# c-f-h/pyiga

Measured on AMD Instinct MI355X. Metric: assembled elements/sec (3D p=4, 128^3 spans) + HBM-roofline %; 1/2/4/8 GPU, higher is better.
Workload: dtype f64

## Files before the change

include/igx.h:

```cpp
#ifndef IGX_H
#define IGX_H

#include <stddef.h>
#include <stdint.h>

#ifdef __cplusplus
extern "C" {
#endif

#define IGX_VERSION 101
#define IGX_MAX_DIM 3
#define IGX_MAX_DEGREE 15
#define IGX_MAX_SF_DEGREE 7

typedef struct igx_ctx igx_ctx;
typedef struct igx_patch igx_patch;
typedef struct igx_multipatch igx_multipatch;

enum { IGX_MASS = 0, IGX_STIFFNESS = 1,
       IGX_CONVDIFF = 2,
       IGX_FORM = 3 };
enum { IGX_GEO_BSPLINE = 0, IGX_GEO_NURBS = 1, IGX_GEO_JACOBIAN = 2 };
enum { IGX_ALGO_AUTO = 0,
       IGX_ALGO_ENTRYWISE = 1,
// ... 21 lines not shown
    const double *gauss_w;

    int32_t row0_lo, row0_hi;

    int32_t box_lo[IGX_MAX_DIM], box_hi[IGX_MAX_DIM];
} igx_patch_desc;

typedef struct {
    int32_t dim, nqp;
    int32_t ndofs[IGX_MAX_DIM], nspans[IGX_MAX_DIM], ngauss[IGX_MAX_DIM];
    int64_t nrows_total;
    int64_t row_lo, row_hi;
    int64_t nnz;
    int64_t nnz_offset;
    int64_t nelem_owned;
    int32_t sumfact_ok;
    int32_t reserved;
} igx_patch_info;

typedef struct {
    float total_ms;
    float fields_ms, stage0_ms, stage1_ms, final_ms, entry_ms;
    int32_t algo_used;
    int32_t n_launches;
} igx_timing;

#define IGX_PATH_GEOA    1
#define IGX_PATH_FUSED   2
#define IGX_PATH_MIRROR  4
#define IGX_PATH_SINGLE  8
#define IGX_PATH_BOTH   32
#define IGX_PATH_BF3    64
#define IGX_PATH_TWIN  128
#define IGX_PATH_KRON   16

int         igx_version(void);
const char *igx_last_error(void);

igx_ctx *igx_create(int device_id);
void     igx_destroy(igx_ctx *ctx);
int      igx_sync(igx_ctx *ctx);
void    *igx_stream(igx_ctx *ctx);

int igx_active_deriv(igx_ctx *ctx, const double *kv, int kv_len, int p,
                     const double *u, size_t nu, int numderiv, double *out);
int igx_find_spans(igx_ctx *ctx, const double *kv, int kv_len, int p,
                   const double *u, size_t nu, int64_t *spans);

int igx_grid_jacobian(igx_ctx *ctx, const igx_patch_desc *desc, int ncomp,
                      const double *const grid[IGX_MAX_DIM], const int32_t ngrid[IGX_MAX_DIM],
                      double *jac_out, double *eval_out);

igx_patch *igx_patch_create(igx_ctx *ctx, const igx_patch_desc *desc);
void       igx_patch_destroy(igx_patch *patch);
int        igx_patch_get_info(const igx_patch *patch, igx_patch_info *info);

int igx_patch_set_coeff(igx_patch *patch, const double *coeff);
int igx_patch_set_coeff_affine(igx_patch *patch, const double c[4]);

int igx_patch_set_coeff_expr(igx_patch *patch, const char *expr, int *cache_hit);

int igx_patch_eval_expr_d(igx_patch *patch, const char *expr, int parametric, double *d_out, int *cache_hit);

int igx_rtc_compile(const char *expr, const char *arch, char *path_out, int path_len, int *cache_hit);

int igx_patch_set_form(igx_patch *patch, const double *const coef[16]);
// ... 397 lines not shown
```

pyiga_amd/assemblers.py:

```python
import os
import ctypes as C
import weakref

import numpy as np
import scipy.sparse

from . import _lib
from . import bspline
from .quadrature import make_tensor_quadrature
from . import geometry

_ENTRY_TRAMPOLINES = []


def _is_spline_geo(geo):
    return hasattr(geo, 'kvs') and hasattr(geo, 'coeffs') and hasattr(geo, 'sdim')


def _is_nurbs(geo):
    from .geometry import NurbsFunc
    return isinstance(geo, NurbsFunc) or type(geo).__name__ == 'NurbsFunc'


class DevicePatch:
# ... 211 lines not shown
            _lib.check(lib.igx_patch_add_face(self.handle, int(axis), int(side), face.handle), 'igx_patch_add_face')
        else:
            vals = _lib.f64(face).ravel()
            _lib.check(lib.igx_patch_add_face_host(self.handle, int(axis), int(side), _lib.dptr(vals), C.c_int64(vals.size)),
                       'igx_patch_add_face_host')

    def assemble_kron(self, kind, patch2, m0, k0=None, to_host=True):
        out = np.empty(self.nnz) if to_host else None
        m0 = _lib.f64(m0)
        k0 = None if k0 is None else _lib.f64(k0)
        _lib.check(_lib.load().igx_assemble_kron3(self.handle, patch2.handle, _lib.KINDS[kind], _lib.dptr(m0),
                                                  None if k0 is None else _lib.dptr(k0), _lib.dptr(out) if to_host else None),
                   'igx_assemble_kron3')
        return out

    def fast_assemble(self, kind, tol=1e-10, maxiter=100, skipcount=3, tolcount=3, verbose=0, batch=None):
        assert self.row_range == (0, self.shape[0]), 'the low-rank assembler works on whole patches'
        lib = _lib.load()
        if batch is not None:
            _lib.check(lib.igx_patch_set_aca_batch(self.handle, int(batch)), 'igx_patch_set_aca_batch')
        data = np.empty(self.nnz)
        rank, nent, nreq = C.c_int(0), C.c_longlong(0), C.c_longlong(0)
        _lib.check(lib.igx_fast_assemble(self.handle, _lib.KINDS[kind], float(tol), int(maxiter), int(skipcount), int(tolcount),
                                         int(verbose), _lib.dptr(data), C.byref(rank), C.byref(nent)), 'igx_fast_assemble')
        _lib.check(lib.igx_fast_assemble_stats(self.handle, C.byref(nreq), None, None), 'igx_fast_assemble_stats')
        self.aca_stats = {'rank': rank.value, 'entries': nent.value, 'requests': nreq.value, 'nnz': int(self.nnz)}
        indptr, indices = self.pattern()
        return scipy.sparse.csr_matrix((data, indices, indptr), shape=self.shape)

    def last_path(self):
        bits = _lib.load().igx_patch_last_path(self.handle)
        return {name for bit, name in ((1, 'geoA'), (2, 'fused'), (4, 'mirror'), (8, 'single'), (16, 'kron'), (32, 'both'), (64, 'bf3'), (128, 'twin')) if bits & bit}

    def fields_plan(self, kind):
        out = (C.c_int64 * 4)()
        _lib.check(_lib.load().igx_patch_fields_plan(self.handle, _lib.KINDS[kind], out), 'igx_patch_fields_plan')
        return {'lines': bool(out[0]), 'lpb': int(out[1]), 'lds': int(out[2]), 'nc': int(out[3])}

    def single2d_plan(self, kind, whole_patch=False):
        out = (C.c_int64 * 9)()
        _lib.check(_lib.load().igx_patch_single2d_plan(self.handle, _lib.KINDS[kind], 1 if whole_patch else 0, out), 'igx_patch_single2d_plan')
        names = ('supported', 'wanted', 'R0', 'R1', 'NG0', 'WIN', 'NCOL', 'lds', 'blocks')
        d = {n: int(v) for n, v in zip(names, out)}
        d['supported'], d['wanted'] = bool(d['supported']), bool(d['wanted'])
        return d

    def placement(self):
        n, b, w = C.c_int(0), C.c_float(0), C.c_float(0)
        _lib.check(_lib.load().igx_patch_placement(self.handle, C.byref(n), C.byref(b), C.byref(w)), 'igx_patch_placement')
        return {'tried': n.value, 'best_ms': round(b.value, 4), 'worst_ms': round(w.value, 4)}

    def timing(self):
        t = _lib.Timing()
        _lib.check(_lib.load().igx_last_timing(self.handle, C.byref(t)), 'igx_last_timing')
        return t.as_dict()

    def entries(self, kind, idx):
        idx = np.ascontiguousarray(idx, dtype=np.uintp)
        assert idx.ndim == 2 and idx.shape[1] == 2
        out = np.zeros(idx.shape[0])
        _lib.check(_lib.load().igx_entries(self.handle, _lib.KINDS[kind], idx.ctypes.data_as(C.POINTER(C.c_size_t)),
                                           idx.shape[0], _lib.dptr(out)), 'igx_entries')
        return out

    def fields(self, kind):
        shp = (C.c_int64 * 4)()
# ... 885 lines not shown
```

pyiga_amd/csrc/geoa.hip:

```cpp
#include <cstdlib>
#include <cstdio>
#include <algorithm>
#include "geo_device.h"

namespace igx {

constexpr int GA_MAXS = 8;
#ifndef GA_ONEDIV
#define GA_ONEDIV 1
#endif
#ifndef GA_SPREAD
#define GA_SPREAD 0
#endif
#ifndef GA_READBOTH
#define GA_READBOTH 1
#endif
#ifndef GA_DPP
#define GA_DPP 1
#endif
typedef const double __attribute__((address_space(4))) *cdp;
typedef const int __attribute__((address_space(4))) *cip;

struct GeoAArgs {
    GeoView gv;
    const double *w0, *w1, *w2;
    int nurbs, kind;
    int G1, G2;
    long long NPL, stride;
    const double *tab;
    const int *steps;
    int s_lo, s_hi, q, chunk_len;
    int ntiles;
#ifdef IGX_ABLATE
    int dbg;
#endif
    int field[GA_MAXS], type[GA_MAXS];
    double *out[GA_MAXS];
    int xfield[GA_MAXS], xtype[GA_MAXS];
    const double *coeff;
    int g0_lo, coef_affine;
    double cf[4];
    int soff_ok;
    double pc[16];
    const double *pa[16];
    int pmask, amask, fmask;
    int fslot[16];
    int nsrc[GA_MAXS], sfield[GA_MAXS][4], stype[GA_MAXS][4];
    int nslots;
    int nodiag[GA_MAXS];
};
constexpr int GA_NFT = 13;

typedef int int8v __attribute__((ext_vector_type(8)));

#ifdef IGX_ABLATE
#define GA_OFF(bit) (A.dbg & (bit))
#else
#define GA_OFF(bit) false
#endif

#ifdef IGX_GA_STAMP
__device__ unsigned long long g_ga_stamp[2048 * 8 * 6];
#define GA_T(i) do { const unsigned long long n_ = __builtin_amdgcn_s_memtime(); st_[i] += n_ - st_t; st_t = n_; } while (0)
#else
#define GA_T(i)
#endif

template <int M>
__device__ __forceinline__ void fmac_rowbc(double &acc, const double pv, const double bv)
{
    asm("v_fmac_f64_dpp %0, %1, %2 row_newbcast:%3 row_mask:0xf bank_mask:0xf" : "+v"(acc) : "v"(pv), "v"(bv), "n"(M));
}
template <int P, int A_ = 0, int B_ = 0>
__device__ __forceinline__ void sweep_lower_rowbc(double (&acc)[P][P], const double (&pv)[(P * (P + 1) / 2 + 15) / 16], const double bv)
{
    if constexpr (A_ < P) {
        constexpr int m = A_ * (A_ + 1) / 2 + B_;
        fmac_rowbc<(m & 15)>(acc[A_][B_], pv[m >> 4], bv);
        if constexpr (B_ < A_) sweep_lower_rowbc<P, A_, B_ + 1>(acc, pv, bv);
        else sweep_lower_rowbc<P, A_ + 1, 0>(acc, pv, bv);
    }
}

template <int P, int M = 0>
__device__ __forceinline__ void sweep_full_rowbc(double (&acc)[P][P], const double (&pv)[(P * P + 15) / 16], const double bv)
{
    if constexpr (M < P * P) {
        fmac_rowbc<(M & 15)>(acc[M / P][M % P], pv[M >> 4], bv);
        sweep_full_rowbc<P, M + 1>(acc, pv, bv);
    }
}

constexpr int GA_REC = 42;
constexpr int GA_ROWS = 16;

__global__ void k_geoa_table(const double *V0s, int P, const double *V0g, const int *fa0g, int P0G, const double *w0, int q,
                             const int *step_ptr, const int *steps, int G0, double *tab, const int *rows, int nonsym)
{
    const int g = blockIdx.x * blockDim.x + threadIdx.x;
    if (g >= G0) return;
    double *r = tab + (size_t)g * GA_REC;
    for (int k = 0; k < GA_REC; ++k) r[k] = 0.0;
    for (int a = 0; a < P; ++a) { r[a] = V0s[((size_t)g * P + a) * 2]; r[6 + a] = V0s[((size_t)g * P + a) * 2 + 1]; }
    for (int e = 0; e < 2 * P0G; ++e) r[12 + e] = V0g[(size_t)g * P0G * 2 + e];
    r[18] = w0[g];
    r[19] = (double)fa0g[g];
    int *ri = (int *)(r + 20);
    const int s = g / q;
    if (g - s * q == q - 1) {
        const int st0 = step_ptr[s], st1 = step_ptr[s + 1];
        ri[0] = st1 - st0; ri[1] = st0;
        if (st1 > st0 && !nonsym)
            for (int a = 0; a < P; ++a) ri[2 + a] = steps[(size_t)st0 * 8 + a];
    }
    int *ra = (int *)(r + 24), *rs = (int *)(r + 32), *rb = (int *)(r + 40);
    for (int m = 0; m < GA_ROWS; ++m) { ra[m] = 0; rs[m] = -1; }
    rb[0] = 0; rb[1] = 0;
    if (nonsym) {
        if (g - s * q == q - 1 && step_ptr[s + 1] > step_ptr[s])
            for (int m = 0; m < 16; ++m) ra[m] = steps[(size_t)step_ptr[s] * 16 + m];
    } else if (rows) {
        const int *sr = rows + (size_t)s * (2 * GA_ROWS + 2);
        for (int m = 0; m < GA_ROWS; ++m) ra[m] = sr[m];
        if (g - s * q == q - 1) {
            for (int m = 0; m < GA_ROWS; ++m) rs[m] = sr[GA_ROWS + m];
            rb[0] = sr[2 * GA_ROWS];
        }
    }
}

struct K1Store {
    __amdgpu_buffer_rsrc_t rs;
    int voff, ok;
    int voffd, nodiag;
    __device__ __forceinline__ K1Store(double *base, const long long pt, const int tile, const int soff_ok, const int nodiag_ = 0)
    {
        const long long t0 = (long long)tile * 64;
        rs = __builtin_amdgcn_make_buffer_rsrc((void *)(base + t0), (short)0, 0x7ffffff0, 0x00020000);
        voff = (int)(pt - t0) * 8;
        nodiag = nodiag_;
        voffd = nodiag_ ? 0x7ffffff8 : voff;
#ifdef GA_K1_FLAT
        ok = 0;
#else
        ok = soff_ok;
#endif
    }
    __device__ __forceinline__ void store(double *out, const int slot, const long long stride, const double x) const
    {
        if (ok) {
            typedef int i2s __attribute__((ext_vector_type(2)));
            i2s v; v.x = __double2loint(x); v.y = __double2hiint(x);
            __builtin_amdgcn_raw_buffer_store_b64(v, rs, voff, (int)((unsigned)slot * (unsigned)(stride * 8)), 0);
        } else out[(long long)slot * stride] = x;
    }
    __device__ __forceinline__ void store_diag(double *out, const int slot, const long long stride, const double x) const
    {
        if (ok) {
            typedef int i2s __attribute__((ext_vector_type(2)));
            i2s v; v.x = __double2loint(x); v.y = __double2hiint(x);
            __builtin_amdgcn_raw_buffer_store_b64(v, rs, voffd, (int)((unsigned)slot * (unsigned)(stride * 8)), 0);
        } else if (!nodiag) out[(long long)slot * stride] = x;
// ... 769 lines not shown
            __syncthreads();
        }
        return;
    }
    if constexpr (DPS) {
        const bool live = w < A.nslots;
        const int t = A.type[w], fi = A.field[w];
        double *const out = A.out[w] + pt;
        const K1Store k1s(A.out[w], pt, tile, A.soff_ok, D2 ? 0 : A.nodiag[w]);
        double acc[P][P];
#pragma unroll
        for (int a = 0; a < P; ++a)
#pragma unroll
            for (int b = 0; b < P; ++b) acc[a][b] = 0.0;
        auto products = [&](const int rsl, const int bufn) {
            for (int i = tid; i < NS * 64; i += NT) {
                const int jp = i >> 6, ty = (i >> 4) & 3, m = i & 15;
                const int a = m >= 10 ? 4 : m >= 6 ? 3 : m >= 3 ? 2 : m >= 1 ? 1 : 0, b = m - a * (a + 1) / 2;
                const double x = rec[rsl][jp][6 * (ty >> 1) + a] * rec[rsl][jp][6 * (ty & 1) + b];
                prd_[((bufn * NS + jp) * 4 + ty) * 16 + m] = m < NPR ? x : 0.0;
            }
        };
        const double *const pw = &prd_[t * 16 + (lane & 15)];
#ifdef IGX_GA_STAMP
        unsigned long long st_[6] = {0, 0, 0, 0, 0, 0}, st_t = __builtin_amdgcn_s_memtime();
#endif
        stage_load(g_begin); stage_store(0);
        stage_load(g_begin + NS); stage_store(1);
        __syncthreads();
        next_batch(g_begin, 0, 0);
        products(0, 0);
        __syncthreads();
        GA_T(0);
        int it = 0, l = 0, sp = s_begin, rs = 0;
        for (int gb = g_begin; gb < g_end; gb += NS, ++it) {
            const int buf = it & 1;
            const int rn = rs == 2 ? 0 : rs + 1, ra = rn == 2 ? 0 : rn + 1;
            stage_load(gb + 2 * NS);
            double pv[1] = {pw[(buf * NS) * 64]};
            double bv = FLD(buf, 0, fi, lane);
#pragma unroll
            for (int j = 0; j < NS; ++j) {
                if (gb + j >= g_end || !live) break;
                const int jn = j + 1 < NS ? j + 1 : j;
                const double pvn = pw[(buf * NS + jn) * 64], bvn = FLD(buf, jn, fi, lane);
                asm volatile("" ::: "memory");
                if (!GA_OFF(4)) sweep_lower_rowbc<P>(acc, pv, bv);
                else acc[0][0] += pv[0] + bv;
#pragma unroll
                for (int a = 0; a < P; ++a)
#pragma unroll
                    for (int b = 0; b <= a; ++b) asm volatile("" : "+v"(acc[a][b]));
                asm volatile("" ::: "memory");
                pv[0] = pvn; bv = bvn;
                GA_T(1);
                if (++l < q) continue;
                const bool write = sp >= own_lo && !GA_OFF(2);
                const int *fr = (const int *)&rec[rs][j][20];
                const int nst = __builtin_amdgcn_readfirstlane(fr[0]), st0 = __builtin_amdgcn_readfirstlane(fr[1]);
                for (int st = st0; st < st0 + nst; ++st) {
                    int pr[P];
                    if (st == st0) {
#pragma unroll
                        for (int a = 0; a < P; ++a) pr[a] = __builtin_amdgcn_readfirstlane(fr[2 + a]);
                    } else {
                        const int8v rec8 = *(const int8v __attribute__((address_space(4))) *)((cip)A.steps + (size_t)st * 8);
#pragma unroll
                        for (int a = 0; a < P; ++a) pr[a] = rec8[a];
                    }
                    if (pr[0] >= 0 && write) k1s.store_diag(out, pr[0], A.stride, acc[0][0]);
#pragma unroll
                    for (int a = 1; a < P; ++a)
                        if (pr[a] >= 0 && write) k1s.store(out, pr[a], A.stride, acc[a][0]);
#pragma unroll
                    for (int a = 0; a < P - 1; ++a)
#pragma unroll
                        for (int b = 0; b <= a; ++b) acc[a][b] = acc[a + 1][b + 1];
#pragma unroll
                    for (int b = 0; b < P; ++b) acc[P - 1][b] = 0.0;
                }
                l = 0; ++sp;
                GA_T(2);
            }
            GA_T(1);
            next_batch(gb + NS, rn, buf ^ 1);
            products(rn, buf ^ 1);
            GA_T(0);
            stage_store(ra);
            rs = rn;
            __syncthreads();
            GA_T(3);
        }
#ifdef IGX_GA_STAMP
        if (lane == 0 && blockIdx.x < 2048 && blockIdx.y == 0)
            for (int i = 0; i < 4; ++i) g_ga_stamp[(blockIdx.x * 8 + (w & 7)) * 6 + i] = st_[i];
#endif
        return;
    }
    const int t = A.type[w], fi = A.field[w];
    double *const out = A.out[w] + pt;
    const K1Store k1s(A.out[w], pt, tile, A.soff_ok);
    double acc[P][P];
#pragma unroll
    for (int a = 0; a < P; ++a)
#pragma unroll
        for (int b = 0; b < P; ++b) acc[a][b] = 0.0;
#if GA_SPREAD
    double park[P];
    int pslot[P];
    bool have = false;
#pragma unroll
    for (int a = 0; a < P; ++a) { park[a] = 0.0; pslot[a] = -1; }
#endif
    typedef double d2 __attribute__((ext_vector_type(2)));
    const int tu = t & 1, tv = t >> 1;
    auto basis_row = [&](double (&v)[PV], const int buf, const int j, const int d) {
        const d2 *row = (const d2 *)&rec[buf][j][6 * d];
#pragma unroll
        for (int k = 0; k < P / 2; ++k) { const d2 x = row[k]; v[2 * k] = x.x; v[2 * k + 1] = x.y; }
        if (P & 1) v[P - 1] = rec[buf][j][6 * d + P - 1];
    };

#ifdef IGX_GA_STAMP
    unsigned long long st_[6] = {0, 0, 0, 0, 0, 0}, st_t = __builtin_amdgcn_s_memtime();
#endif
// ... 75 lines not shown
                if (nst == 1 && gb + j + 1 < g_end) {
#pragma unroll
                    for (int a = 0; a < P; ++a) { park[a] = acc[a][0]; pslot[a] = write ? pr[a] : -1; }
                    have = true;
                } else
#endif
#pragma unroll
                for (int a = 0; a < P; ++a)
                    if (pr[a] >= 0 && write) k1s.store(out, pr[a], A.stride, acc[a][0]);
#pragma unroll
                for (int a = 0; a < P - 1; ++a)
#pragma unroll
                    for (int b = 0; b <= a; ++b) acc[a][b] = acc[a + 1][b + 1];
#pragma unroll
                for (int b = 0; b < P; ++b) acc[P - 1][b] = 0.0;
            }
            l = 0; ++sp;
            GA_T(2);
        }
        GA_T(1);
        next_batch(gb + NS, rn, buf ^ 1);
        GA_T(0);
        stage_store(ra);
        rs = rn;
        __syncthreads();
        GA_T(3);
    }
#ifdef IGX_GA_STAMP
    if (lane == 0 && blockIdx.x < 2048 && blockIdx.y == 0)
        for (int i = 0; i < 4; ++i) g_ga_stamp[(blockIdx.x * 8 + (w & 7)) * 6 + i] = st_[i];
#endif
}

template <int P, int NS, int P0G>
static int launch_geoA_2d(hipStream_t st, const GeoAArgs &A, int nc, dim3 grid)
{
    if (nc == 3) k_geoA<P, NS, P0G, 3, false, 0, true><<<grid, dim3(geoa_threads(NS, 0)), 0, st>>>(A);
    else k_geoA<P, NS, P0G, 2, false, 0, true><<<grid, dim3(geoa_threads(NS, 0)), 0, st>>>(A);
    IGX_HIP(hipGetLastError());
    return IGX_OK;
}

template <int P, int NS, int P0G, bool MF = false, int FORM = 0>
static int launch_geoA_k(hipStream_t st, const GeoAArgs &A, int nc, dim3 grid)
{
    if (nc == 4) k_geoA<P, NS, P0G, 4, MF, FORM><<<grid, dim3(geoa_threads(NS, FORM)), 0, st>>>(A);
    else k_geoA<P, NS, P0G, 3, MF, FORM><<<grid, dim3(geoa_threads(NS, FORM)), 0, st>>>(A);
    IGX_HIP(hipGetLastError());
#ifdef IGX_GA_STAMP
    {
        static std::vector<unsigned long long> h(2048 * 8 * 6);
        IGX_HIP(hipStreamSynchronize(st));
        IGX_HIP(hipMemcpyFromSymbol(h.data(), HIP_SYMBOL(g_ga_stamp), h.size() * sizeof(unsigned long long)));
        const int nb = std::min<unsigned>(grid.x, 2048);
        for (int w = 0; w < NS; ++w) {
            double t[4] = {0, 0, 0, 0};
            for (int b = 0; b < nb; ++b) for (int i = 0; i < 4; ++i) t[i] += h[(b * 8 + w) * 6 + i];
            fprintf(stderr, "k_geoA stamp: wave %d  geometry %.0f  sweep %.0f  flush %.0f  barrier %.0f  (x100 ns per block)\n", w, t[0] / nb, t[1] / nb, t[2] / nb, t[3] / nb);
        }
    }
#endif
    return IGX_OK;
}

template <int P, int NS>
static int launch_geoA_g(hipStream_t st, const GeoAArgs &A, int nc, int p0g, dim3 grid)
// ... 109 lines not shown
        hipError_t e = hipGetLastError();
        if (e == hipSuccess) e = hipStreamSynchronize(st);
        (void)hipFree(d_rows);
        if (e != hipSuccess) {
            (void)hipFree(tab);
            set_error("per-plane table of the fused geometry + axis-0 sweep: %s", hipGetErrorString(e));
            return IGX_ERR_HIP;
        }
        pt->d_geoa_tab = tab;
        pt->geoa_mf = mf_ok ? 1 : 0;
    }
    GeoAArgs A{};
    const bool d2 = pt->dim == 2;
    A.gv = make_view(pt->dim, pt->gax, pt->d_ctrl, pt->ncomp);
    A.w0 = pd.ax[0].w; A.w1 = pd.ax[1].w; A.w2 = d2 ? nullptr : pd.ax[2].w;
    A.nurbs = pt->geo_kind == IGX_GEO_NURBS; A.kind = kind;
    A.G1 = pd.ax[1].G; A.G2 = d2 ? 1 : pd.ax[2].G;
    A.NPL = (long long)A.G1 * A.G2; A.stride = slice_stride;
    A.soff_ok = (long long)(nonsym ? pt->npairs0n : pt->npairs0) * slice_stride * 8 + 1024 < 0x7ffffff0LL ? 1 : 0;
    A.tab = nonsym ? pt->d_geoa_tabn : pt->d_geoa_tab; A.steps = nonsym ? pt->d_stepsn : pt->stepA_rec;
    A.coeff = pt->d_coeff; A.g0_lo = pd.g0_lo; A.coef_affine = pt->coef_affine;
    for (int k = 0; k < 4; ++k) A.cf[k] = pt->coef_c[k];
    A.s_lo = pt->s0_lo; A.s_hi = pt->s0_hi; A.q = A0.q; A.chunk_len = chunk_len;
#ifdef IGX_ABLATE
    { const char *e = getenv("IGX_GEOA_DBG"); A.dbg = e ? atoi(e) : 0; }
#endif
    for (int x = 0; x < nslots; ++x) {
        A.field[x] = slot_field ? slot_field[x] : 0; A.type[x] = slot_type ? slot_type[x] : 0; A.out[x] = slot_out[x];
        A.xfield[x] = slot_xfield ? slot_xfield[x] : -1; A.xtype[x] = slot_xtype ? slot_xtype[x] : 0;
        A.nodiag[x] = (nodiag_mask >> x) & 1;
    }
    if (nodiag_mask && (nonsym || form || pt->dim != 3 || !geoA_diag_types_commute(pt))) { set_error("internal: diagonal slices skipped on a sweep that does not repeat them"); return IGX_ERR_UNSUPPORTED; }
    A.nslots = nslots;
    for (int x = nslots; x < GA_MAXS; ++x) A.out[x] = A.out[0];
    A.ntiles = (int)((A.NPL + 63) / 64);
    dim3 grid((unsigned)((A.ntiles + 7) / 8 * 8), nchunks);
    const int nc = pt->ncomp, p0g = pt->gax[0].P;
    if (d2) {
#define GEOA_2D(PV) case PV: return nslots == 1 ? (p0g == 2 ? launch_geoA_2d<PV, 1, 2>(st, A, nc, grid) : launch_geoA_2d<PV, 1, 3>(st, A, nc, grid)) \
                                                : (p0g == 2 ? launch_geoA_2d<PV, 4, 2>(st, A, nc, grid) : launch_geoA_2d<PV, 4, 3>(st, A, nc, grid))
        switch (A0.P) { GEOA_2D(2); GEOA_2D(3); GEOA_2D(4); GEOA_2D(5); }
#undef GEOA_2D
        set_error("fused geometry + stage A (2D): unsupported degree %d", A0.p);
        return IGX_ERR_UNSUPPORTED;
    }
    if (form) {
        for (int k = 0; k < 16; ++k) { A.pc[k] = form->pc[k]; A.pa[k] = form->pa[k]; A.fslot[k] = form->fslot[k]; }
        A.pmask = form->pmask; A.nslots = nslots; A.amask = 0; A.fmask = 0;
        for (int k = 0; k < 16; ++k) { if (form->pa[k]) A.amask |= 1 << k; if (form->fslot[k] >= 0) A.fmask |= 1 << k; }
        for (int x = 0; x < GA_MAXS; ++x) {
            A.nsrc[x] = x < nslots ? form->nsrc[x] : 1;
            for (int k = 0; k < 4; ++k) { A.sfield[x][k] = x < nslots ? form->sfield[x][k] : 0; A.stype[x][k] = x < nslots ? form->stype[x][k] : 0; }
            if (x >= nslots) A.out[x] = A.out[0];
        }
#define GEOA_T(PV, FV) case PV: return p0g == 2 ? launch_geoA_k<PV, 8, 2, false, FV>(st, A, nc, grid) : p0g == 3 ? launch_geoA_k<PV, 8, 3, false, FV>(st, A, nc, grid) : IGX_ERR_UNSUPPORTED
        if (form->sym) switch (A0.P) { GEOA_T(3, 3); GEOA_T(4, 3); GEOA_T(5, 3); GEOA_T(6, 3); }
        else switch (A0.P) { GEOA_T(3, 2); GEOA_T(4, 2); GEOA_T(5, 2); GEOA_T(6, 2); }
#undef GEOA_T
        set_error("fused geometry + stage A (general form): unsupported degree %d", A0.p);
        return IGX_ERR_UNSUPPORTED;
    }
    if (nonsym) {
#define GEOA_N(PV) case PV: return p0g == 2 ? launch_geoA_k<PV, 8, 2, false, 1>(st, A, nc, grid) : p0g == 3 ? launch_geoA_k<PV, 8, 3, false, 1>(st, A, nc, grid) : IGX_ERR_UNSUPPORTED
        switch (A0.P) {
            GEOA_N(3); GEOA_N(4); GEOA_N(5); GEOA_N(6);
        }
#undef GEOA_N
        set_error("fused geometry + stage A (non-symmetric): unsupported degree %d", A0.p);
        return IGX_ERR_UNSUPPORTED;
    }
    if (nslots == 8 && pt->geoa_mf && pt->knobs.geoa_mf && (A0.P == 5 || A0.P == 4) && A0.q == A0.P && p0g == 2) {
        if (A0.P == 5) return launch_geoA_k<5, 8, 2, true>(st, A, nc, grid);
        return launch_geoA_k<4, 8, 2, true>(st, A, nc, grid);
    }
#define GEOA_P(PV) case PV: return (nslots == 1 && !(GA_MASS8 && PV <= 5)) ? launch_geoA_g<PV, 1>(st, A, nc, p0g, grid) : launch_geoA_g<PV, 8>(st, A, nc, p0g, grid)
    switch (A0.P) {
        GEOA_P(2); GEOA_P(3); GEOA_P(4); GEOA_P(5); GEOA_P(6);
    }
#undef GEOA_P
    set_error("fused geometry + stage A: unsupported degree %d", A0.p);
    return IGX_ERR_UNSUPPORTED;
}

}
```

pyiga_amd/csrc/igx_api.hip:

```cpp
#include "igx_internal.h"
#include <algorithm>
#include <cmath>
#include <cstdarg>
#include <cstdio>
#include <cstdlib>
#include <cstring>
#include <new>

namespace igx {

static thread_local char g_err[1024] = "";

void set_error(const char *fmt, ...)
{
    va_list ap;
    va_start(ap, fmt);
    vsnprintf(g_err, sizeof(g_err), fmt, ap);
    va_end(ap);
}

static void gauss_legendre(int n, std::vector<double> &x, std::vector<double> &w)
{
    x.assign(n, 0.0);
    w.assign(n, 0.0);
// ... 355 lines not shown
    (void)hipSetDevice(pt->ctx->device);
    (void)hipStreamSynchronize(pt->ctx->stream);
    for (int k = 0; k < 3; ++k) { free_axis(pt->ax[k]); free_geo_axis(pt->gax[k]); }
    (void)hipFree(pt->d_ctrl); (void)hipFree(pt->d_jac); (void)hipFree(pt->d_coeff); (void)hipFree(pt->d_formc); (void)hipFree(pt->d_fields); (void)hipFree(pt->d_data);
    (void)hipFree(pt->ftab_arr);
    (void)hipFree(pt->d_indices); (void)hipFree(pt->d_indptr); (void)hipFree(pt->d_pl0); (void)hipFree(pt->d_rl0_of); (void)hipFree(pt->d_steps); (void)hipFree(pt->d_ldesc);
    (void)hipFree(pt->d_pl0n); (void)hipFree(pt->d_stepsn); (void)hipFree(pt->d_qdesc); (void)hipFree(pt->d_qdescn);
    (void)hipFree(pt->d_K1); (void)hipFree(pt->d_K2);
    (void)hipFree(pt->d_geoa_tab); (void)hipFree(pt->d_geoa_tabn); (void)hipFree(pt->d_zeros); (void)hipFree(pt->d_triv); (void)hipFree(pt->d_tpairs);
    (void)hipFree(pt->d_ws_ij); (void)hipFree(pt->d_ws_out);
    (void)hipFree(pt->d_lv_f); (void)hipFree(pt->d_lv_t1); (void)hipFree(pt->d_lv_t2); (void)hipFree(pt->d_lv_o);
    (void)hipFree(pt->d_sp_ws);
    (void)hipFree(pt->d_q_ws);
    delete pt;
}

igx_patch *igx_patch_create(igx_ctx *ctx, const igx_patch_desc *d)
{
    if (!ctx || !d) { set_error("igx_patch_create: null argument"); return nullptr; }
    const int dim = d->dim;
    if (dim != 2 && dim != 3) { set_error("igx_patch_create: dim must be 2 or 3 (got %d)", dim); return nullptr; }
    if (hipSetDevice(ctx->device) != hipSuccess) { set_error("hipSetDevice failed"); return nullptr; }
    igx_patch *pt = new (std::nothrow) igx_patch();
    if (pt) {
        igx_knobs &k = pt->knobs;
        if (const char *e = getenv("IGX_PATH")) k.path = !strcmp(e, "fused") ? 1 : !strcmp(e, "unfused") ? 2 : !strcmp(e, "single") ? 3 : 0;
        if (const char *e = getenv("IGX_GEOA")) { k.geoa = strcmp(e, "0") != 0; k.geoa_mf = strcmp(e, "mfma") == 0; }
        if (const char *e = getenv("IGX_FINAL")) k.final_sel = !strcmp(e, "q") ? 1 : !strcmp(e, "valu") ? 2 : !strcmp(e, "mfma") ? 3 : 1;
        if (const char *e = getenv("IGX_ENTRIES")) k.entries_thread = !strcmp(e, "thread");
        k.poison = getenv("IGX_DEBUG_POISON") != nullptr;
        if (const char *e = getenv("IGX_BF")) k.bf = atoi(e);
        k.no_twin = getenv("IGX_NO_TWIN") != nullptr;
        if (const char *e = getenv("IGX_NO_DIAG_SKIP")) k.no_diag_skip = strcmp(e, "0") != 0;
        if (const char *e = getenv("IGX_PLACEMENT_TRIES")) k.placement_tries = std::max(1, std::min(16, atoi(e)));
        if (const char *e = getenv("IGX_STAGE_EVENTS")) k.stage_events = strcmp(e, "0") != 0;
    }
    if (pt) for (int k = 0; k < 16; ++k) pt->form_slot[k] = -1;
    if (!pt) return nullptr;
    pt->ctx = ctx;
    pt->dim = dim;
    hipStream_t st = ctx->stream;
    int rc = IGX_OK;

    int q = d->nqp;
    if (q <= 0) { q = 0; for (int k = 0; k < dim; ++k) q = std::max(q, d->p[k] + 1); }
    pt->nqp = q;
    std::vector<double> gx, gw;
    if (d->gauss_x && d->gauss_w) { gx.assign(d->gauss_x, d->gauss_x + q); gw.assign(d->gauss_w, d->gauss_w + q); }
    else gauss_legendre(q, gx, gw);

    for (int k = 0; k < dim && !rc; ++k) {
        if (!d->kv[k]) { set_error("igx_patch_create: kv[%d] is null", k); rc = IGX_ERR_ARG; break; }
        rc = setup_axis(pt->ax[k], d->kv[k], d->kv_len[k], d->p[k], q, gx.data(), gw.data());
        if (!rc) rc = upload_axis(pt->ax[k], st);
    }
    if (dim == 2) {
        pt->ax[2].N = 1; pt->ax[2].n = 1; pt->ax[2].G = 1; pt->ax[2].S = 1; pt->ax[2].q = q;
        pt->ax[2].dev.N = 1; pt->ax[2].dev.n = 1; pt->ax[2].dev.G = 1; pt->ax[2].dev.S = 1; pt->ax[2].dev.q = q;
    }
    if (!rc && pt->knobs.stage_events < 0) {
        long long npts = 1;
        for (int k = 0; k < dim; ++k) npts *= pt->ax[k].G;
        pt->knobs.stage_events = dim == 3 && npts >= (1ll << 24);
    }
    for (int k = 0; k < dim && !rc; ++k) pt->boxed = pt->boxed || d->box_hi[k] != 0 || d->box_lo[k] != 0;
    if (!rc && pt->boxed) {
// ... 1139 lines not shown
```

pyiga_amd/csrc/igx_internal.h:

```cpp
#pragma once
#include <hip/hip_runtime.h>
#include <stdint.h>
#include <stddef.h>
#include <string>
#include <vector>
#include "igx.h"

namespace igx {

constexpr int MAXP = IGX_MAX_DEGREE + 1;
constexpr int MAX_COMP = 4;

void set_error(const char *fmt, ...);
#define IGX_HIP(call)                                                                   \
    do {                                                                                \
        hipError_t e_ = (call);                                                         \
        if (e_ != hipSuccess) {                                                         \
            igx::set_error("%s:%d: %s -> %s", __FILE__, __LINE__, #call, hipGetErrorString(e_)); \
            return IGX_ERR_HIP;                                                         \
        }                                                                               \
    } while (0)

struct AxisDev {
    int p, P, N, n, q, G;
// ... 50 lines not shown
    double *d_kv = nullptr, *d_nodes = nullptr, *d_w = nullptr, *d_V = nullptr, *d_PI = nullptr;
    int *d_ints = nullptr;
    int ord[2] = {0, 1};
    AxisDev dev{};
};

struct GeoAxis {
    int p = 0, P = 0, N = 0;
    std::vector<double> kv;
    double *d_kv = nullptr;
    double *d_V = nullptr;
    int *d_fa = nullptr;
};

}

struct igx_ctx {
    int device = 0;
    int ncu = 0;
    hipStream_t stream = nullptr;
    hipEvent_t ev[8] = {};
};

struct igx_knobs {
    int path = 0;
    int geoa = 1;
    int geoa_mf = 0;
    int final_sel = 0;
    int entries_thread = 0;
    int poison = 0;
    int bf = 0;
    int no_twin = 0;
    int no_diag_skip = 0;
    int placement_tries = 1;
    int stage_events = -1;
};

struct igx_patch;
static inline void stage_event(const igx_patch *pt, int k, hipStream_t st);

struct igx_patch {
    igx_ctx *ctx = nullptr;
    igx_knobs knobs;
    bool basis_default = true;
    bool boxed = false;
    int dim = 0, nqp = 0;
    igx::Axis ax[3];
    int geo_kind = 0, ncomp = 0;
    igx::GeoAxis gax[3];
    double *d_ctrl = nullptr;
    double *d_jac = nullptr;
    double *d_formc = nullptr;
    int form_slot[16];
    void *form_fn = nullptr;
    struct FormTable {
        bool valid = false, sym = false, blocksym = false;
        int present = 0, is_const = 0;
        double cval[16] = {0};
        std::string expr[16];
        int arr_of[16];
        int narr = 0;
    } ftab;
    double *ftab_arr = nullptr;
    bool ftab_ready = false;
    igx_patch *twin = nullptr;
    int twin_kinds = 0;
// ... 254 lines not shown
```

Before: 179.1 million.

## Rotate geoA accumulator window by phase instead of shifting registers per span

At each span end, the geoA kernel used to shift the triangular accumulator array down by one row and column, which costs many register moves. It now keeps a compile-time phase and indexes the accumulators through a rotating window. A goto-based state machine dispatches the phase per plane, and the extra multi-step stores are deferred to a tail loop. Explicit kernel instantiations are moved into a separate translation unit so the two builds can compile in parallel. This enlarges code size and branch complexity, and it is gated on simple symmetric cases with P up to 5.

Result: faster. 181.1 million, median of 6 (+1.1%).

```diff
diff --git a/include/igx.h b/include/igx.h
--- a/include/igx.h
+++ b/include/igx.h
@@ -77,6 +77,7 @@
 #define IGX_PATH_BOTH   32
 #define IGX_PATH_BF3    64
 #define IGX_PATH_TWIN  128
+#define IGX_PATH_GEOA_ROT 256
 #define IGX_PATH_KRON   16
 
 int         igx_version(void);
diff --git a/pyiga_amd/assemblers.py b/pyiga_amd/assemblers.py
--- a/pyiga_amd/assemblers.py
+++ b/pyiga_amd/assemblers.py
@@ -267,6 +267,9 @@
         bits = _lib.load().igx_patch_last_path(self.handle)
         return {name for bit, name in ((1, 'geoA'), (2, 'fused'), (4, 'mirror'), (8, 'single'), (16, 'kron'), (32, 'both'), (64, 'bf3'), (128, 'twin')) if bits & bit}
 
+    def geoa_rotated(self):
+        return bool(_lib.load().igx_patch_last_path(self.handle) & 256)
+
     def fields_plan(self, kind):
         out = (C.c_int64 * 4)()
         _lib.check(_lib.load().igx_patch_fields_plan(self.handle, _lib.KINDS[kind], out), 'igx_patch_fields_plan')
diff --git a/pyiga_amd/csrc/geoa.hip b/pyiga_amd/csrc/geoa.hip
--- a/pyiga_amd/csrc/geoa.hip
+++ b/pyiga_amd/csrc/geoa.hip
@@ -1,6 +1,7 @@
 #include <cstdlib>
 #include <cstdio>
 #include <algorithm>
+#include <type_traits>
 #include "geo_device.h"
 
 namespace igx {
@@ -48,6 +49,7 @@
     int nsrc[GA_MAXS], sfield[GA_MAXS][4], stype[GA_MAXS][4];
     int nslots;
     int nodiag[GA_MAXS];
+    int rot;
 };
 constexpr int GA_NFT = 13;
 
@@ -60,6 +62,9 @@
 #endif
 
 #ifdef IGX_GA_STAMP
+#ifdef GEOA_SYM_TU
+extern
+#endif
 __device__ unsigned long long g_ga_stamp[2048 * 8 * 6];
 #define GA_T(i) do { const unsigned long long n_ = __builtin_amdgcn_s_memtime(); st_[i] += n_ - st_t; st_t = n_; } while (0)
 #else
@@ -71,15 +76,29 @@
 {
     asm("v_fmac_f64_dpp %0, %1, %2 row_newbcast:%3 row_mask:0xf bank_mask:0xf" : "+v"(acc) : "v"(pv), "v"(bv), "n"(M));
 }
-template <int P, int A_ = 0, int B_ = 0>
+template <int P, int PH>
+__device__ __forceinline__ double &win_acc(double (&acc)[P][P], const int a, const int b)
+{
+    const int r = (PH + a) % P, c = (PH + b) % P;
+    return acc[r > c ? r : c][r > c ? c : r];
+}
+template <int P, int A_ = 0, int B_ = 0, int PH = 0>
 __device__ __forceinline__ void sweep_lower_rowbc(double (&acc)[P][P], const double (&pv)[(P * (P + 1) / 2 + 15) / 16], const double bv)
 {
     if constexpr (A_ < P) {
         constexpr int m = A_ * (A_ + 1) / 2 + B_;
-        fmac_rowbc<(m & 15)>(acc[A_][B_], pv[m >> 4], bv);
-        if constexpr (B_ < A_) sweep_lower_rowbc<P, A_, B_ + 1>(acc, pv, bv);
-        else sweep_lower_rowbc<P, A_ + 1, 0>(acc, pv, bv);
-    }
+        fmac_rowbc<(m & 15)>(win_acc<P, PH>(acc, A_, B_), pv[m >> 4], bv);
+        if constexpr (B_ < A_) sweep_lower_rowbc<P, A_, B_ + 1, PH>(acc, pv, bv);
+        else sweep_lower_rowbc<P, A_ + 1, 0, PH>(acc, pv, bv);
+    }
+}
+template <int P, int PH = 0, class F>
+__device__ __forceinline__ bool with_phase(const int phase, F &&f)
+{
+    if constexpr (PH + 1 < P) {
+        if (phase != PH) return with_phase<P, PH + 1>(phase, f);
+    }
+    return f(std::integral_constant<int, PH>{});
 }
 
 template <int P, int M = 0>
@@ -94,6 +113,7 @@
 constexpr int GA_REC = 42;
 constexpr int GA_ROWS = 16;
 
+#ifndef GEOA_SYM_TU
 __global__ void k_geoa_table(const double *V0s, int P, const double *V0g, const int *fa0g, int P0G, const double *w0, int q,
                              const int *step_ptr, const int *steps, int G0, double *tab, const int *rows, int nonsym)
 {
@@ -128,6 +148,7 @@
         }
     }
 }
+#endif
 
 struct K1Store {
     __amdgpu_buffer_rsrc_t rs;
@@ -963,65 +984,141 @@
         products(0, 0);
         __syncthreads();
         GA_T(0);
-        int it = 0, l = 0, sp = s_begin, rs = 0;
-        for (int gb = g_begin; gb < g_end; gb += NS, ++it) {
-            const int buf = it & 1;
-            const int rn = rs == 2 ? 0 : rs + 1, ra = rn == 2 ? 0 : rn + 1;
-            stage_load(gb + 2 * NS);
-            double pv[1] = {pw[(buf * NS) * 64]};
-            double bv = FLD(buf, 0, fi, lane);
-#pragma unroll
-            for (int j = 0; j < NS; ++j) {
-                if (gb + j >= g_end || !live) break;
-                const int jn = j + 1 < NS ? j + 1 : j;
-                const double pvn = pw[(buf * NS + jn) * 64], bvn = FLD(buf, jn, fi, lane);
-                asm volatile("" ::: "memory");
-                if (!GA_OFF(4)) sweep_lower_rowbc<P>(acc, pv, bv);
-                else acc[0][0] += pv[0] + bv;
-#pragma unroll
-                for (int a = 0; a < P; ++a)
-#pragma unroll
-                    for (int b = 0; b <= a; ++b) asm volatile("" : "+v"(acc[a][b]));
-                asm volatile("" ::: "memory");
-                pv[0] = pvn; bv = bvn;
+        auto batches = [&](auto rotc) __attribute__((always_inline)) {
+            constexpr bool ROT = decltype(rotc)::value;
+            int it = 0, l = 0, sp = s_begin, rs = 0, phase = 0;
+            for (int gb = g_begin; gb < g_end; gb += NS, ++it) {
+                const int buf = it & 1;
+                const int rn = rs == 2 ? 0 : rs + 1, ra = rn == 2 ? 0 : rn + 1;
+                stage_load(gb + 2 * NS);
+                const double *const pwb = pw + (buf * NS) * 64, *const fb = &FLD(buf, 0, fi, lane);
+                double pv[1] = {pwb[0]};
+                double bv = fb[0];
+                auto sweep_plane = [&](auto phc, const int j) __attribute__((always_inline)) {
+                    constexpr int PH = decltype(phc)::value;
+                    const int jn = j + 1 < NS ? j + 1 : j;
+                    const double pvn = pwb[jn * 64], bvn = fb[jn * FST];
+                    asm volatile("" ::: "memory");
+                    if (!GA_OFF(4)) sweep_lower_rowbc<P, 0, 0, PH>(acc, pv, bv);
+                    else acc[0][0] += pv[0] + bv;
+#pragma unroll
+                    for (int a = 0; a < P; ++a)
+#pragma unroll
+                        for (int b = 0; b <= a; ++b) asm volatile("" : "+v"(acc[a][b]));
+                    asm volatile("" ::: "memory");
+                    pv[0] = pvn; bv = bvn;
+                    GA_T(1);
+                };
+                auto span_end = [&](auto phc, const int j) __attribute__((always_inline)) {
+                    constexpr int PH = decltype(phc)::value;
+                    const bool write = sp >= own_lo && !GA_OFF(2);
+                    const int *fr = (const int *)&rec[rs][j][20];
+                    if constexpr (ROT) {
+                        int pr[P];
+#pragma unroll
+                        for (int a = 0; a < P; ++a) pr[a] = __builtin_amdgcn_readfirstlane(fr[2 + a]);
+                        if (pr[0] >= 0 && write) k1s.store_diag(out, pr[0], A.stride, win_acc<P, PH>(acc, 0, 0));
+#pragma unroll
+                        for (int a = 1; a < P; ++a)
+                            if (pr[a] >= 0 && write) k1s.store(out, pr[a], A.stride, win_acc<P, PH>(acc, a, 0));
+#pragma unroll
+                        for (int a = 0; a < P; ++a) win_acc<P, PH>(acc, a, 0) = 0.0;
+                    } else {
+                        const int nst = __builtin_amdgcn_readfirstlane(fr[0]), st0 = __builtin_amdgcn_readfirstlane(fr[1]);
+                        for (int st = st0; st < st0 + nst; ++st) {
+                            int pr[P];
+                            if (st == st0) {
+#pragma unroll
+                                for (int a = 0; a < P; ++a) pr[a] = __builtin_amdgcn_readfirstlane(fr[2 + a]);
+                            } else {
+                                const int8v rec8 = *(const int8v __attribute__((address_space(4))) *)((cip)A.steps + (size_t)st * 8);
+#pragma unroll
+                                for (int a = 0; a < P; ++a) pr[a] = rec8[a];
+                            }
+                            if (pr[0] >= 0 && write) k1s.store_diag(out, pr[0], A.stride, acc[0][0]);
+#pragma unroll
+                            for (int a = 1; a < P; ++a)
+                                if (pr[a] >= 0 && write) k1s.store(out, pr[a], A.stride, acc[a][0]);
+#pragma unroll
+                            for (int a = 0; a < P - 1; ++a)
+#pragma unroll
+                                for (int b = 0; b <= a; ++b) acc[a][b] = acc[a + 1][b + 1];
+#pragma unroll
+                            for (int b = 0; b < P; ++b) acc[P - 1][b] = 0.0;
+                        }
+                    }
+                    l = 0; ++sp;
+                    GA_T(2);
+                };
+                if constexpr (ROT) {
+#define GA_ROT_PLANE(PH, J, PHN, JN) \
+                    ga_##PH##_##J: \
+                    if constexpr (PH < P && J < NS) { \
+                        if (J >= nj) { phase = PH; goto ga_done; } \
+                        sweep_plane(std::integral_constant<int, PH>{}, J); \
+                        if (++l < q) goto ga_##PH##_##JN; \
+                        span_end(std::integral_constant<int, PH>{}, J); \
+                        if constexpr (PH + 1 == P) goto ga_0_##JN; else goto ga_##PHN##_##JN; \
+                    } else if constexpr (PH < P && J == NS) { phase = PH; goto ga_done; }
+#define GA_ROT_ROW(J, JN) GA_ROT_PLANE(0, J, 1, JN) GA_ROT_PLANE(1, J, 2, JN) GA_ROT_PLANE(2, J, 3, JN) GA_ROT_PLANE(3, J, 4, JN) GA_ROT_PLANE(4, J, 0, JN)
+                    static_assert(P <= 5 && NS <= 8, "phases and planes of the table below");
+                    {
+                        const int nj = live ? g_end - gb : 0;
+                        if (phase == 1) goto ga_1_0;
+                        if (phase == 2) goto ga_2_0;
+                        if (phase == 3) goto ga_3_0;
+                        if (phase == 4) goto ga_4_0;
+                        goto ga_0_0;
+                        GA_ROT_ROW(0, 1) GA_ROT_ROW(1, 2) GA_ROT_ROW(2, 3) GA_ROT_ROW(3, 4)
+                        GA_ROT_ROW(4, 5) GA_ROT_ROW(5, 6) GA_ROT_ROW(6, 7) GA_ROT_ROW(7, 8)
+                        ga_0_8: phase = 0; goto ga_done;
+                        ga_1_8: phase = 1; goto ga_done;
+                        ga_2_8: phase = 2; goto ga_done;
+                        ga_3_8: phase = 3; goto ga_done;
+                        ga_4_8: phase = 4;
+                        ga_done:;
+                    }
+#undef GA_ROT_ROW
+#undef GA_ROT_PLANE
+                } else {
+#pragma unroll
+                    for (int j = 0; j < NS; ++j) {
+                        if (gb + j >= g_end || !live) break;
+                        sweep_plane(std::integral_constant<int, 0>{}, j);
+                        if (++l < q) continue;
+                        span_end(std::integral_constant<int, 0>{}, j);
+                    }
+                }
                 GA_T(1);
-                if (++l < q) continue;
-                const bool write = sp >= own_lo && !GA_OFF(2);
-                const int *fr = (const int *)&rec[rs][j][20];
-                const int nst = __builtin_amdgcn_readfirstlane(fr[0]), st0 = __builtin_amdgcn_readfirstlane(fr[1]);
-                for (int st = st0; st < st0 + nst; ++st) {
-                    int pr[P];
-                    if (st == st0) {
-#pragma unroll
-                        for (int a = 0; a < P; ++a) pr[a] = __builtin_amdgcn_readfirstlane(fr[2 + a]);
-                    } else {
+                next_batch(gb + NS, rn, buf ^ 1);
+                products(rn, buf ^ 1);
+                GA_T(0);
+                stage_store(ra);
+                rs = rn;
+                __syncthreads();
+                GA_T(3);
+            }
+            if constexpr (ROT) {
+                if (live && g_end > g_begin && own_hi > own_lo && !GA_OFF(2)) {
+                    cip fr = (cip)(const int *)(A.tab + (size_t)g_last * GA_REC + 20);
+                    const int nst = fr[0], st0 = fr[1];
+                    for (int st = st0 + 1; st < st0 + nst; ++st) {
                         const int8v rec8 = *(const int8v __attribute__((address_space(4))) *)((cip)A.steps + (size_t)st * 8);
-#pragma unroll
-                        for (int a = 0; a < P; ++a) pr[a] = rec8[a];
+                        with_phase<P>(phase, [&](auto phc) __attribute__((always_inline)) -> bool {
+                            constexpr int PH = decltype(phc)::value;
+                            if (rec8[0] >= 0) k1s.store_diag(out, rec8[0], A.stride, win_acc<P, PH>(acc, 0, 0));
+#pragma unroll
+                            for (int a = 1; a < P; ++a)
+                                if (rec8[a] >= 0) k1s.store(out, rec8[a], A.stride, win_acc<P, PH>(acc, a, 0));
+                            return true;
+                        });
+                        phase = phase + 1 == P ? 0 : phase + 1;
                     }
-                    if (pr[0] >= 0 && write) k1s.store_diag(out, pr[0], A.stride, acc[0][0]);
-#pragma unroll
-                    for (int a = 1; a < P; ++a)
-                        if (pr[a] >= 0 && write) k1s.store(out, pr[a], A.stride, acc[a][0]);
-#pragma unroll
-                    for (int a = 0; a < P - 1; ++a)
-#pragma unroll
-                        for (int b = 0; b <= a; ++b) acc[a][b] = acc[a + 1][b + 1];
-#pragma unroll
-                    for (int b = 0; b < P; ++b) acc[P - 1][b] = 0.0;
                 }
-                l = 0; ++sp;
-                GA_T(2);
-            }
-            GA_T(1);
-            next_batch(gb + NS, rn, buf ^ 1);
-            products(rn, buf ^ 1);
-            GA_T(0);
-            stage_store(ra);
-            rs = rn;
-            __syncthreads();
-            GA_T(3);
-        }
+            }
+        };
+        if (A.rot) batches(std::true_type{});
+        else batches(std::false_type{});
 #ifdef IGX_GA_STAMP
         if (lane == 0 && blockIdx.x < 2048 && blockIdx.y == 0)
             for (int i = 0; i < 4; ++i) g_ga_stamp[(blockIdx.x * 8 + (w & 7)) * 6 + i] = st_[i];
@@ -1163,6 +1260,20 @@
 #endif
 }
 
+#ifdef GEOA_SYM_TU
+#define GEOA_DPS_INST(...) template __global__ void k_geoA<__VA_ARGS__>(const GeoAArgs);
+#else
+#define GEOA_DPS_INST(...) extern template __global__ void k_geoA<__VA_ARGS__>(const GeoAArgs);
+#endif
+#define GEOA_DPS_NC(PV, NSV, GV, NC0, NC1, D2V) GEOA_DPS_INST(PV, NSV, GV, NC0, false, 0, D2V) GEOA_DPS_INST(PV, NSV, GV, NC1, false, 0, D2V)
+#define GEOA_DPS_P(PV) GEOA_DPS_NC(PV, 1, 2, 3, 4, false) GEOA_DPS_NC(PV, 1, 3, 3, 4, false) GEOA_DPS_NC(PV, 8, 2, 3, 4, false) GEOA_DPS_NC(PV, 8, 3, 3, 4, false) \
+                       GEOA_DPS_NC(PV, 1, 2, 2, 3, true) GEOA_DPS_NC(PV, 1, 3, 2, 3, true) GEOA_DPS_NC(PV, 4, 2, 2, 3, true) GEOA_DPS_NC(PV, 4, 3, 2, 3, true)
+GEOA_DPS_P(2) GEOA_DPS_P(3) GEOA_DPS_P(4) GEOA_DPS_P(5)
+#undef GEOA_DPS_P
+#undef GEOA_DPS_NC
+#undef GEOA_DPS_INST
+
+#ifndef GEOA_SYM_TU
 template <int P, int NS, int P0G>
 static int launch_geoA_2d(hipStream_t st, const GeoAArgs &A, int nc, dim3 grid)
 {
@@ -1338,11 +1449,13 @@
     }
     if (nodiag_mask && (nonsym || form || pt->dim != 3 || !geoA_diag_types_commute(pt))) { set_error("internal: diagonal slices skipped on a sweep that does not repeat them"); return IGX_ERR_UNSUPPORTED; }
     A.nslots = nslots;
+    A.rot = GA_DPP && A0.simple && !pt->knobs.no_geoa_rot && A0.P * (A0.P + 1) / 2 <= 16;
     for (int x = nslots; x < GA_MAXS; ++x) A.out[x] = A.out[0];
     A.ntiles = (int)((A.NPL + 63) / 64);
     dim3 grid((unsigned)((A.ntiles + 7) / 8 * 8), nchunks);
     const int nc = pt->ncomp, p0g = pt->gax[0].P;
     if (d2) {
+        if (A.rot) pt->last_path |= IGX_PATH_GEOA_ROT;
 #define GEOA_2D(PV) case PV: return nslots == 1 ? (p0g == 2 ? launch_geoA_2d<PV, 1, 2>(st, A, nc, grid) : launch_geoA_2d<PV, 1, 3>(st, A, nc, grid)) \
                                                 : (p0g == 2 ? launch_geoA_2d<PV, 4, 2>(st, A, nc, grid) : launch_geoA_2d<PV, 4, 3>(st, A, nc, grid))
         switch (A0.P) { GEOA_2D(2); GEOA_2D(3); GEOA_2D(4); GEOA_2D(5); }
@@ -1379,6 +1492,7 @@
         if (A0.P == 5) return launch_geoA_k<5, 8, 2, true>(st, A, nc, grid);
         return launch_geoA_k<4, 8, 2, true>(st, A, nc, grid);
     }
+    if (A.rot) pt->last_path |= IGX_PATH_GEOA_ROT;
 #define GEOA_P(PV) case PV: return (nslots == 1 && !(GA_MASS8 && PV <= 5)) ? launch_geoA_g<PV, 1>(st, A, nc, p0g, grid) : launch_geoA_g<PV, 8>(st, A, nc, p0g, grid)
     switch (A0.P) {
         GEOA_P(2); GEOA_P(3); GEOA_P(4); GEOA_P(5); GEOA_P(6);
@@ -1387,5 +1501,6 @@
     set_error("fused geometry + stage A: unsupported degree %d", A0.p);
     return IGX_ERR_UNSUPPORTED;
 }
+#endif
 
 }
diff --git a/pyiga_amd/csrc/geoa_sym.hip b/pyiga_amd/csrc/geoa_sym.hip
--- /dev/null
+++ b/pyiga_amd/csrc/geoa_sym.hip
@@ -0,0 +1,2 @@
+#define GEOA_SYM_TU
+#include "geoa.hip"
diff --git a/pyiga_amd/csrc/igx_api.hip b/pyiga_amd/csrc/igx_api.hip
--- a/pyiga_amd/csrc/igx_api.hip
+++ b/pyiga_amd/csrc/igx_api.hip
@@ -411,6 +411,7 @@
         if (const char *e = getenv("IGX_BF")) k.bf = atoi(e);
         k.no_twin = getenv("IGX_NO_TWIN") != nullptr;
         if (const char *e = getenv("IGX_NO_DIAG_SKIP")) k.no_diag_skip = strcmp(e, "0") != 0;
+        if (const char *e = getenv("IGX_NO_GEOA_ROT")) k.no_geoa_rot = strcmp(e, "0") != 0;
         if (const char *e = getenv("IGX_PLACEMENT_TRIES")) k.placement_tries = std::max(1, std::min(16, atoi(e)));
         if (const char *e = getenv("IGX_STAGE_EVENTS")) k.stage_events = strcmp(e, "0") != 0;
     }
diff --git a/pyiga_amd/csrc/igx_internal.h b/pyiga_amd/csrc/igx_internal.h
--- a/pyiga_amd/csrc/igx_internal.h
+++ b/pyiga_amd/csrc/igx_internal.h
@@ -106,6 +106,7 @@
     int bf = 0;
     int no_twin = 0;
     int no_diag_skip = 0;
+    int no_geoa_rot = 0;
     int placement_tries = 1;
     int stage_events = -1;
 };
```
